# arindamrc/video_analytics

Measured on AMD Instinct MI355X. Metric: clips/sec (224x224, RGB+10-flow two-stream), higher is better.
Workload: dtype f32; 1 GPU; two-stream 224x224, 10-frame TV-L1 flow stack (5 scales x 5 warps x 300 its, fixed), VGG-16 spatial+temporal, batch=32 per GPU; global_batch=32, block_iters=0, tvl1_math=exact, flow_streams=2, batches_in_flight=1, tvl1_params=, tvl1_hip_blob=20e9f45376b19dd960a619139aafc0e8722a8659, parallelism=clips sharded x1, finite=True

## Files before the change

include/va.h:

```cpp
#ifndef VA_H
#define VA_H

#include <stddef.h>
#include <stdint.h>

#ifdef __cplusplus
extern "C" {
#endif

#define VA_OK 0
#define VA_ERR_INVALID 1
#define VA_ERR_HIP 2
#define VA_ERR_WORKSPACE 3
#define VA_ERR_STOPPED 4

#define VA_DTYPE_F32 0
#define VA_DTYPE_BF16 1

typedef struct va_ctx va_ctx;
typedef struct va_vgg16 va_vgg16;

#define VA_VERSION_EXPERIMENTS 0x10000
int va_version(void);
const char* va_last_error(void);
// ... 1 lines not shown
void va_ctx_destroy(va_ctx* ctx);


int va_vgg16_create(va_ctx* ctx, int c_in, int n_classes, int desc_dim, int dtype,
                    const void* const* conv_w, const void* const* conv_b,
                    const void* const* fc_w, const void* const* fc_b,
                    const float* in_mean, const float* in_std,
                    void* stream, va_vgg16** out);
void va_vgg16_destroy(va_vgg16* model);
size_t va_vgg16_workspace_bytes(const va_vgg16* model, int batch);

#define VA_OPT_BF16_VARIANT 1
#define VA_OPT_F32_CONV_KERNEL 2
#define VA_OPT_TRAIN_STOP_AT 3
#define VA_OPT_BF16_FIRST_LAYER 4
int va_vgg16_set_option(va_vgg16* model, int option, int value);

int va_vgg16_forward(va_vgg16* model, const void* x, int x_is_u8, int batch,
                     void* feat, void* desc, void* logits,
                     void* workspace, size_t workspace_bytes, void* stream);

int va_vgg16_classify(va_vgg16* model, const void* feat, int batch, void* desc, void* logits,
                      void* workspace, size_t workspace_bytes, void* stream);

int va_copy_first_layer(va_ctx* ctx, const void* w_rgb, int cout, int n_in, void* w_out, void* stream);

int va_validate_batch(va_ctx* ctx, const void* logits, const void* labels, int batch, int n_classes,
                      void* out, void* stream);


typedef struct va_tvl1_params {
    float tau;
    float lambda;
    float theta;
    int nscales;
// ... 53 lines not shown

int va_flow_motion(va_ctx* ctx, const void* flow, int n_chains, int chain_len, int trajectory, int w, int h,
                   const void* means, void* out, void* stream);

int va_flow_homography(va_ctx* ctx, const void* flow, int n_fields, int w, int h, int iters, double c0_sq, double cmin_sq,
                       void* H, void* stats, void* stream);

int va_flow_compensate(va_ctx* ctx, const void* flow, int n_fields, int w, int h, const void* H, void* out, void* stream);

int va_selftest_exact_math(va_ctx* ctx, float lo, float hi, unsigned long long* mismatches, void* stream);


int va_conv3x3_layer(va_ctx* ctx, int dtype, int kernel_opt, int hw, int cin_pad, int cout, int pool, int linear,
                     int out_f32, int batch, const void* in, const void* w_packed, const float* bias, const float* mask,
                     const void* zeros, void* out, char* kernel_name, int name_len, void* stream);

int va_train_conv_backward_layer(va_ctx* ctx, int kernel_opt, int batch, int hw, int cin, int cin_pad, int cout,
                                 const float* dy, const float* x, float* w_packed, float* bias, float* mom_w, float* mom_b,
                                 float lr, float momentum, float* dx, const float* mask, const float* zeros, float* slab,
                                 float* wt, float* bpart, size_t* scratch_floats, char* info, int info_len, void* stream);
int va_train_fc_backward_layer(va_ctx* ctx, int batch, int out_f, int in_f, const float* dz, const float* x, float* w,
                               float* bias, float* mom_w, float* mom_b, float lr, float momentum, float* dx,
                               const float* mask, float scale, char* info, int info_len, void* stream);
int va_train_pool_layer(va_ctx* ctx, int batch, int hw, int c, const float* y, float* p, const float* dp, float* dy,
                        void* stream);
int va_train_loss(va_ctx* ctx, const float* logits, const void* labels, int n, int k, int c, float* dlogits, float* out,
                  void* stream);
int va_train_loss_multitask(va_ctx* ctx, const float* logits, const void* labels, const void* tasks, int n, int k,
                            int n_heads, const int* head_sizes, float* dlogits, float* out, void* stream);
int va_train_dropout(va_ctx* ctx, float* x, size_t n, unsigned long long dropout_seed, int layer, void* stream);
// ... 54 lines not shown
```

video_analytics_amd/_ffi.py:

```python
import ctypes
import os

_HERE = os.path.dirname(os.path.abspath(__file__))
LIB_PATH = os.path.join(_HERE, "libva_hip.so")

VA_OK, VA_ERR_INVALID, VA_ERR_HIP, VA_ERR_WORKSPACE, VA_ERR_STOPPED = 0, 1, 2, 3, 4
VA_OPT_BF16_VARIANT, VA_OPT_F32_CONV_KERNEL, VA_OPT_TRAIN_STOP_AT, VA_OPT_BF16_FIRST_LAYER = 1, 2, 3, 4

EXPORTS = [
    "va_version", "va_last_error", "va_ctx_create", "va_ctx_destroy",
    "va_vgg16_create", "va_vgg16_destroy", "va_vgg16_workspace_bytes", "va_vgg16_set_option", "va_vgg16_forward", "va_vgg16_classify",
    "va_copy_first_layer", "va_validate_batch",
    "va_tvl1_default_params", "va_tvl1_pyramid_sizes", "va_tvl1_tile_plan", "va_tvl1_workspace_bytes", "va_tvl1_flow",
    "va_flow_to_stack", "va_flow_to_stack_crop", "va_crop_images_u8",
    "va_flow_to_stack_views", "va_crop_images_u8_views", "va_view_mean", "va_flow_field_means", "va_flow_motion",
    "va_selftest_exact_math", "va_tvl1_profile_enable", "va_tvl1_profile_read", "va_tvl1_profile_levels",
    "va_flow_to_stack_snippets", "va_score_consensus", "va_fuse_scores",
    "va_meter_update", "va_meter_average", "va_linear_svm_predict",
    "va_vgg16_train_init", "va_vgg16_train_workspace_bytes", "va_vgg16_train_step",
    "va_vgg16_export_state", "va_vgg16_import_state", "va_vgg16_train_plan",
    "va_conv3x3_layer",
    "va_flow_to_stack_resize", "va_resize_images_u8", "va_vgg16_train_step_consensus",
    "va_flow_homography", "va_flow_compensate",
    "va_rgbdiff_to_stack", "va_fuse_scores_n",
    "va_train_conv_backward_layer", "va_train_fc_backward_layer", "va_train_pool_layer", "va_train_loss", "va_train_dropout",
    "va_vgg16_train_step_multitask", "va_train_loss_multitask",
    "va_linear_svm_fit_workspace_bytes", "va_linear_svm_fit", "va_linear_svm_fit_cg_steps",
]


TUNING_SLOTS = ("stream_levels", "stream_waves", "stream_chunks", "stream_slots", "rows_levels", "stream_ppl",
                "stream_queue", "rows_cfg")
VA_VERSION_EXPERIMENTS = 0x10000


class Tvl1Params(ctypes.Structure):
    _fields_ = [
        ("tau", ctypes.c_float),
        ("lambda_", ctypes.c_float),
        ("theta", ctypes.c_float),
        ("nscales", ctypes.c_int),
        ("warps", ctypes.c_int),
# ... 42 lines not shown
    L.va_last_error.restype = ctypes.c_char_p
    L.va_ctx_create.argtypes = [ci, pp]
    L.va_ctx_create.restype = ci
    L.va_ctx_destroy.argtypes = [vp]
    L.va_ctx_destroy.restype = None
    L.va_vgg16_create.argtypes = [vp, ci, ci, ci, ci, pp, pp, pp, pp, fpp, fpp, vp, pp]
    L.va_vgg16_create.restype = ci
    L.va_vgg16_destroy.argtypes = [vp]
    L.va_vgg16_destroy.restype = None
    L.va_vgg16_workspace_bytes.argtypes = [vp, ci]
    L.va_vgg16_workspace_bytes.restype = sz
    L.va_vgg16_set_option.argtypes = [vp, ci, ci]
    L.va_vgg16_set_option.restype = ci
    L.va_vgg16_forward.argtypes = [vp, vp, ci, ci, vp, vp, vp, vp, sz, vp]
    L.va_vgg16_forward.restype = ci
    L.va_vgg16_classify.argtypes = [vp, vp, ci, vp, vp, vp, sz, vp]
    L.va_vgg16_classify.restype = ci
    L.va_copy_first_layer.argtypes = [vp, vp, ci, ci, vp, vp]
    L.va_copy_first_layer.restype = ci
    L.va_validate_batch.argtypes = [vp, vp, vp, ci, ci, vp, vp]
    L.va_validate_batch.restype = ci
    L.va_tvl1_default_params.argtypes = [ctypes.POINTER(Tvl1Params)]
    L.va_tvl1_default_params.restype = None
    L.va_tvl1_pyramid_sizes.argtypes = [ci, ci, ctypes.POINTER(Tvl1Params), ctypes.POINTER(ci), ctypes.POINTER(ci)]
    L.va_tvl1_pyramid_sizes.restype = ci
    L.va_tvl1_tile_plan.argtypes = [ci, ci, ctypes.POINTER(Tvl1Params), ctypes.POINTER(ci)]
    L.va_tvl1_tile_plan.restype = ci
    L.va_tvl1_workspace_bytes.argtypes = [ci, ci, ci, ci, ctypes.POINTER(Tvl1Params)]
    L.va_tvl1_workspace_bytes.restype = sz
    L.va_tvl1_flow.argtypes = [vp, vp, ci, ci, ci, ci, ci, ctypes.POINTER(Tvl1Params), vp, vp, sz, vp]
# ... 141 lines not shown
```

video_analytics_amd/csrc/vgg.hip:

```cpp
#include "vgg_internal.h"
#include <cstdint>
#include <cstdlib>
#include <cstring>
#include <type_traits>

namespace {

typedef float f32x16 __attribute__((ext_vector_type(16)));
typedef float f32x4 __attribute__((ext_vector_type(4)));
typedef unsigned u32x4 __attribute__((ext_vector_type(4)));

template <int N, typename F>
__device__ __forceinline__ void static_for(F&& f)
{
    if constexpr (N > 0) {
        static_for<N - 1>(f);
        f(std::integral_constant<int, N - 1>{});
    }
}

constexpr int kBK = 16;
constexpr int kLdsStride = 20;


// ... 1571 lines not shown
                } else {
#pragma unroll
                    for (int j = 0; j < 4; ++j) {
                        const int xx = x + (j & 1), yy = y + (j >> 1);
                        if (xx < W && yy < H) {
                            const size_t o = (((size_t)b * H + yy) * W + xx) * a.Cout + n;
                            a.out[o] = (a.mask && !(a.mask[o] > 0.0f)) ? 0.0f : v[j];
                        }
                    }
                }
            }
        }
    }
}



struct FcArgs {
    const float* A;
    const float* Wt;
    float* slab;
    int M, N, K, S, kchunk, Npad;
};

constexpr int kFcDepth = 4;
__global__ void __launch_bounds__(256) k_fc_splitk(FcArgs a)
{
    __shared__ __attribute__((aligned(16))) float sA[2][32 * kLdsStride];
    __shared__ __attribute__((aligned(16))) float sB[2][128 * kLdsStride];
    const int tid = threadIdx.x, lane = tid & 63, wave = tid >> 6;
// ... 225 lines not shown
        VA_LAUNCHED(pool ? "k_conv3x3_mfma<2,2,2,2,true,16>" : "k_conv3x3_mfma<2,2,2,2,false,16>");
    } else {
        a.tiles_n = cout / 64;
        const unsigned grid = (unsigned)(a.tiles_n * a.tiles_x * a.tiles_y * tiles_b);
        if (pool) k_conv3x3_mfma<2, 2, 2, 1, true, 16><<<grid, 256, 0, st>>>(a);
        else k_conv3x3_mfma<2, 2, 2, 1, false, 16><<<grid, 256, 0, st>>>(a);
        VA_LAUNCHED(pool ? "k_conv3x3_mfma<2,2,2,1,true,16>" : "k_conv3x3_mfma<2,2,2,1,false,16>");
    }
    VA_LAUNCH_CHECK();
    return VA_OK;
}

int launch_conv(const ConvLayer& L, const float* zeros, const float* in, float* out, int B, int f32_conv, hipStream_t st)
{
    return launch_conv_ex(L.hw, L.cin_pad, L.cout, L.wp, L.bias, in, out, nullptr, 0, L.pool, B, zeros, f32_conv, st);
}

int launch_conv_bf16(const ConvLayer& L, const __bf16* zeros, int variant, const __bf16* in, void* out, bool out_f32, int B, int n_cu,
                     hipStream_t st, const char** launched = nullptr)
{
    ConvArgsBf a{};
    a.in = in;
    a.zeros = zeros;
    a.taps_x = L.xcol ? 1 : 3;
    a.wp = L.wp_bf;
    a.bias = L.bias;
    a.out = out;
    a.B = B;
    a.H = a.W = L.hw;
    a.Cin = L.cin_pad;
// ... 290 lines not shown
    m->c_in = c_in;
    m->dtype = dtype;
    m->c_in_pad = dtype == VA_DTYPE_BF16 ? 64 : va_cdiv(c_in, VA_CIN_ALIGN) * VA_CIN_ALIGN;
    m->n_classes = n_classes;
    m->desc_dim = desc_dim;
    int hw = 224, cin = c_in, cin_pad = m->c_in_pad;
    int rc = VA_OK;
    auto fail = [&](int code) { va_vgg16_destroy(m); return code; };
    if (hipMalloc(&m->zeros_f32, 512 * sizeof(float)) != hipSuccess || hipMemsetAsync(m->zeros_f32, 0, 512 * sizeof(float), st) != hipSuccess) {
        va_set_error("va_vgg16_create: hipMalloc failed for the zero line");
        return fail(VA_ERR_HIP);
    }
    m->bf16_variant = 0;
    m->bf16_first = 1;
    m->f32_conv = VA_F32_CONV_DEFAULT;
    m->train_stop_at = -1;
    if (dtype == VA_DTYPE_BF16) {
        if (hipMalloc(&m->zeros, 256) != hipSuccess || hipMemsetAsync(m->zeros, 0, 256, st) != hipSuccess) {
            va_set_error("va_vgg16_create: hipMalloc failed for the zero line");
            return fail(VA_ERR_HIP);
        }
    }
    for (int i = 0; i < 13; ++i) {
        ConvLayer& L = m->conv[i];
        L.cin = cin;
        L.cin_pad = cin_pad;
        L.cout = kConvCout[i];
        L.hw = hw;
        L.pool = kConvPool[i];
        const size_t nw = (size_t)L.cout * 9 * L.cin_pad;
        const bool bf = dtype == VA_DTYPE_BF16;
// ... 50 lines not shown
    *out = m;
    return VA_OK;
}

extern "C" void va_vgg16_destroy(va_vgg16* m)
{
    if (!m) return;
    for (int i = 0; i < 13; ++i) {
        if (m->conv[i].wp) (void)hipFree(m->conv[i].wp);
        if (m->conv[i].wp_bf) (void)hipFree(m->conv[i].wp_bf);
        if (m->conv[i].bias) (void)hipFree(m->conv[i].bias);
        if (m->conv[i].mom_w) (void)hipFree(m->conv[i].mom_w);
        if (m->conv[i].mom_b) (void)hipFree(m->conv[i].mom_b);
    }
    if (m->wp_f1) (void)hipFree(m->wp_f1);
    for (int i = 0; i < 4; ++i) {
        if (m->fcw[i]) (void)hipFree(m->fcw[i]);
        if (m->fcb[i]) (void)hipFree(m->fcb[i]);
        if (m->fc_mom_w[i]) (void)hipFree(m->fc_mom_w[i]);
        if (m->fc_mom_b[i]) (void)hipFree(m->fc_mom_b[i]);
    }
    if (m->zeros_f32) (void)hipFree(m->zeros_f32);
    if (m->zeros) (void)hipFree(m->zeros);
    if (m->in_mean) (void)hipFree(m->in_mean);
    if (m->in_std) (void)hipFree(m->in_std);
    delete m;
}

extern "C" size_t va_vgg16_workspace_bytes(const va_vgg16* m, int batch)
{
    if (!m || batch < 1 || batch > 4096) return 0;
    return plan_ws(m, batch).total;
}

extern "C" int va_vgg16_forward(va_vgg16* m, const void* x, int x_is_u8, int batch, void* feat, void* desc, void* logits,
                                void* workspace, size_t workspace_bytes, void* stream)
{
    VA_CHECK_ARG(m != nullptr, "va_vgg16_forward: model is NULL");
    VA_USE_DEVICE(m->ctx);
    VA_CHECK_ARG(x != nullptr && workspace != nullptr, "va_vgg16_forward: NULL input/workspace");
    VA_CHECK_ARG(batch >= 1 && batch <= 4096, "va_vgg16_forward: batch %d out of range [1,4096]", batch);
    VA_CHECK_ARG(!x_is_u8 || (m->in_mean && m->in_std), "va_vgg16_forward: u8 input needs in_mean/in_std at create time");
    VA_CHECK_ARG(((uintptr_t)workspace & 255) == 0, "va_vgg16_forward: workspace must be 256-byte aligned");
    const WsPlan wp = plan_ws(m, batch);
    if (workspace_bytes < wp.total) {
        va_set_error("va_vgg16_forward: workspace too small (%zu < %zu bytes)", workspace_bytes, wp.total);
        return VA_ERR_WORKSPACE;
    }
    hipStream_t st = (hipStream_t)stream;
    char* ws = (char*)workspace;
    float* act[2] = {(float*)(ws + wp.off_act[0]), (float*)(ws + wp.off_act[1])};
    float* slab = (float*)(ws + wp.off_slab);
    float* fcbuf[2] = {(float*)(ws + wp.off_fc[0]), (float*)(ws + wp.off_fc[1])};
    const int B = batch, HW0 = 224 * 224;
// ... 11 lines not shown
        } else if (m->conv[0].xcol) {
            if (x_is_u8)
                k_nchw_to_nhwc_xcol<unsigned char><<<pgrid, 256, 0, st>>>((const unsigned char*)x, (__bf16*)act[1], B, m->c_in, 224, HW0, m->in_mean, m->in_std);
            else
                k_nchw_to_nhwc_xcol<float><<<pgrid, 256, 0, st>>>((const float*)x, (__bf16*)act[1], B, m->c_in, 224, HW0, nullptr, nullptr);
        } else if (x_is_u8)
            k_nchw_to_nhwc_pad<unsigned char, __bf16><<<pgrid, 256, 0, st>>>((const unsigned char*)x, (__bf16*)act[1], B, m->c_in, HW0, m->c_in_pad, m->in_mean, m->in_std);
        else
            k_nchw_to_nhwc_pad<float, __bf16><<<pgrid, 256, 0, st>>>((const float*)x, (__bf16*)act[1], B, m->c_in, HW0, m->c_in_pad, nullptr, nullptr);
        VA_LAUNCH_CHECK();
        for (int i = first; i < 13; ++i) {
            if (int rc = launch_conv_bf16(m->conv[i], m->zeros, m->bf16_variant, (const __bf16*)act[cur], act[cur ^ 1], i == 12, B, m->ctx->n_cu, st)) return rc;
            cur ^= 1;
        }
    } else {
        if (x_is_u8)
            k_nchw_to_nhwc_pad<unsigned char, float><<<pgrid, 256, 0, st>>>((const unsigned char*)x, act[1], B, m->c_in, HW0, m->c_in_pad, m->in_mean, m->in_std);
        else
            k_nchw_to_nhwc_pad<float, float><<<pgrid, 256, 0, st>>>((const float*)x, act[1], B, m->c_in, HW0, m->c_in_pad, nullptr, nullptr);
        VA_LAUNCH_CHECK();
        for (int i = 0; i < 13; ++i) {
            if (int rc = launch_conv(m->conv[i], m->zeros_f32, act[cur], act[cur ^ 1], B, m->f32_conv, st)) return rc;
            cur ^= 1;
        }
    }
    const float* f = act[cur];
    if (feat) {
        const size_t n = (size_t)B * 512 * 49;
        k_nhwc_to_nchw<<<(unsigned)((n + 255) / 256), 256, 0, st>>>(f, (float*)feat, B, 512, 49);
        VA_LAUNCH_CHECK();
    }
    if (desc || logits) return run_classifier(m, f, B, desc, logits, slab, fcbuf, st);
    return VA_OK;
}

extern "C" int va_vgg16_set_option(va_vgg16* m, int option, int value)
{
    VA_CHECK_ARG(m != nullptr, "va_vgg16_set_option: model is NULL");
    switch (option) {
        case VA_OPT_BF16_VARIANT:
            VA_CHECK_ARG((value >= 0 && value <= 2) || (value >= 5 && value <= 7), "va_vgg16_set_option: VA_OPT_BF16_VARIANT must be 0, 1, 2, 5, 6 or 7");
            VA_CHECK_ARG(value != 6 || kVaExperiments, "va_vgg16_set_option: VA_OPT_BF16_VARIANT 6 (k_conv3x3_bpp_bf16) needs a library built with -DVA_EXPERIMENTS");
            m->bf16_variant = value;
            return VA_OK;
        case VA_OPT_BF16_FIRST_LAYER:
            VA_CHECK_ARG(value == 0 || value == 1, "va_vgg16_set_option: VA_OPT_BF16_FIRST_LAYER must be 0 or 1");
            m->bf16_first = value;
            return VA_OK;
        case VA_OPT_F32_CONV_KERNEL:
            VA_CHECK_ARG(value == 0 || value == 1, "va_vgg16_set_option: VA_OPT_F32_CONV_KERNEL must be 0 or 1");
            m->f32_conv = value;
            return VA_OK;
        case VA_OPT_TRAIN_STOP_AT:
            VA_CHECK_ARG(value >= -1 && value <= 12, "va_vgg16_set_option: VA_OPT_TRAIN_STOP_AT must be in [-1,12]");
            m->train_stop_at = value;
            return VA_OK;
        default:
            va_set_error("va_vgg16_set_option: unknown option %d", option);
            return VA_ERR_INVALID;
    }
}

extern "C" int va_vgg16_classify(va_vgg16* m, const void* feat, int batch, void* desc, void* logits, void* workspace,
                                 size_t workspace_bytes, void* stream)
{
    VA_CHECK_ARG(m != nullptr, "va_vgg16_classify: model is NULL");
    VA_USE_DEVICE(m->ctx);
// ... 42 lines not shown
```

video_analytics_amd/csrc/vgg_internal.h:

```cpp
#pragma once
#include "va_internal.h"

struct ConvLayer {
    int cin, cin_pad, cout, hw;
    bool pool;
    bool xcol;
    float* wp;
    __bf16* wp_bf;
    float* bias;
    float* mom_w;
    float* mom_b;
};


struct va_vgg16 {
    va_ctx* ctx;
    int c_in, c_in_pad, n_classes, desc_dim, dtype;
    ConvLayer conv[13];
    float* fcw[4];
    float* fcb[4];
    int fc_in[4], fc_out[4];
    float* in_mean;
    float* in_std;
    __bf16* zeros;
    float* fc_mom_w[4];
    float* fc_mom_b[4];
    float* zeros_f32;
    __bf16* wp_f1;
    int f1_cp, f1_krow;
    int bf16_first;
    int bf16_variant;
    int f32_conv;
    int train_stop_at;
};


int va_conv3x3_f32(int hw, int cin_pad, int cout, const float* wp, const float* bias, const float* in, float* out,
                   const float* mask, int linear, int pool, int B, const float* zeros, int f32_conv, hipStream_t st,
                   const char** launched = nullptr);
int va_fc_f32(const float* A, const float* Wt, const float* bias, float* out, float* slab, int M, int N, int K, int relu, hipStream_t st);
size_t va_fc_slab_floats(int M, int N, int K);
int va_input_to_nhwc_f32(const va_vgg16* m, const void* x, int x_is_u8, int B, float* out, hipStream_t st);

#define VA_MAX_HEADS 8
struct va_heads {
    int n;
    int off[VA_MAX_HEADS + 1];
};
// ... 4 lines not shown
```

video_analytics_amd/pipeline.py:

```python
import torch

from . import flow as vflow
from . import augment, fusion, rgbdiff, synth, vgg, video
from .parameters import (NACTION_CLASSES, NORM_MEANS_TF, NORM_STDS_TF, VIDEO_DESCRIPTOR_DIM,
                         VIDEO_INPUT_FLOW_COUNT)


def build_stream_weights(c_in, seed, device, n_classes=NACTION_CLASSES):
    w = synth.synth_vgg16_weights(c_in=c_in, n_classes=n_classes, desc_dim=VIDEO_DESCRIPTOR_DIM, seed=seed,
                                  device=device)
    if c_in != 3:
        w["conv_w"][0] = vgg.copy_first_layer(w["conv_w"][0].to(device), c_in)
    return w


def check_video(rgb, gray, flow_count, motion, n_snippets, views, consensus, fusion_weights, crops=None):
    if crops is not None:
        raise ValueError("submit_video: a video takes views=, not crops= (one table for all its snippets)")
    if motion != "stack":
        raise ValueError("submit_video: motion=%r is not offered for whole videos (its chains depend on the window); "
                         "use motion='stack'" % (motion,))
    if not isinstance(rgb, torch.Tensor) or rgb.dtype != torch.uint8 or rgb.dim() != 4 or rgb.shape[1] != 3:
        raise ValueError("submit_video: rgb must be a uint8 [T,3,H,W] tensor")
    if not isinstance(gray, torch.Tensor) or gray.dim() != 3 or gray.dtype not in (torch.uint8, torch.float32):
# ... 83 lines not shown

    def _tvl1_frames(self, gray):
        return vflow.bidirectional_sequences(gray) if self.motion == "bidirectional" else gray

    def _camera(self, flow, out):
        if self.camera != "none":
            _, out["homography"], out["camera_share"] = vflow.apply_camera(flow, self.camera, in_place=True)
        return flow

    def _motion_field(self, flow, k):
        if self.motion != "trajectory" and not self.mean_flow:
            return flow
        return vflow.apply_motion(flow, self.L, self.motion, self.mean_flow,
                                  out=self._buffer(self._motion, k, tuple(flow.shape)))

    def _buffer(self, bank, k, shape):
        t = bank[k]
        if t is None or tuple(t.shape) != tuple(shape):
            if t is not None:
                evs = []
                for st in [self._cnn, self._cnn2] + list(vflow.flow_streams(self.device, self.flow_streams)):
                    ev = torch.cuda.Event()
                    ev.record(st)
                    evs.append(ev)
                self._retired.append((t, evs))
            self._retired = [(old, evs) for old, evs in self._retired if not all(e.query() for e in evs)]
            bank[k] = t = torch.empty(shape, dtype=torch.float32, device=self.device)
        return t

    def _check_views(self, rgb, gray, flow_stack, views):
# ... 58 lines not shown
        flow = evs = None
        extra = {}
        if flow_stack is None:
            B, F, H, W = gray.shape
            fbuf = self._buffer(self._flow, k, (B * self.L, 2, H, W))
            flow, evs = vflow.tvl1_flow_concurrent(tv, self.tvl1_params, self.flow_streams, out=fbuf,
                                                   after=[ready, self._flow_read[k]], join=False)
        with torch.cuda.stream(self._cnn):
            self._cnn.wait_event(ready)
            rgb.record_stream(self._cnn)
            _, desc_s, logits_s = self.spatial.forward(rgb if rgb_crops is None else augment.crop_images(rgb, rgb_crops))
            if flow_stack is None:
                for ev in evs:
                    self._cnn.wait_event(ev)
                B, F, H, W = gray.shape
                src = self._motion_field(self._camera(flow, extra), k)
                if flow_crops is None:
                    stack = vflow.flow_to_stack(src, out=self._buffer(self._stack, k, (B, 2 * self.L, H, W)))
                else:
                    stack = vflow.crop_flow_to_stack(src, flow_crops,
                                                     out=self._buffer(self._stack, k, (B, 2 * self.L, 224, 224)),
                                                     invert_x_on_flip=bool(invert_flow_x))
                done = torch.cuda.Event()
                done.record(self._cnn)
                self._flow_read[k] = done
                if self._t_done is not None:
                    self._cnn.wait_event(self._t_done)
                _, desc_t, logits_t = self.temporal.forward(stack)
                self._t_done = torch.cuda.Event()
                self._t_done.record(self._cnn)
            else:
                self._cnn2.wait_event(ready)
                if self._t_done is not None:
                    self._cnn2.wait_event(self._t_done)
                with torch.cuda.stream(self._cnn2):
                    flow_stack.record_stream(self._cnn2)
                    _, desc_t, logits_t = self.temporal.forward(flow_stack)
                    self._t_done = torch.cuda.Event()
                    self._t_done.record(self._cnn2)
                self._cnn.wait_stream(self._cnn2)
            finished = torch.cuda.Event()
            finished.record(self._cnn)
        out = dict(logits_s=logits_s, logits_t=logits_t, desc_s=desc_s, desc_t=desc_t, **extra)
        self._handed_out.extend(out.values())
        out["done"] = finished
# ... 287 lines not shown
```

video_analytics_amd/vgg.py:

```python
import ctypes

import torch

from . import _ffi

_ws_cache = {}


def _workspace(nbytes, device, slot=0):
    key = (device.index, "vgg", slot)
    t = _ws_cache.get(key)
    if t is None or t.numel() < nbytes:
        _ws_cache[key] = t = torch.empty(nbytes, dtype=torch.uint8, device=device)
    return t


def release_workspaces():
    _ws_cache.clear()


def copy_first_layer(w_rgb, n_in):
    if not w_rgb.is_cuda or w_rgb.dtype != torch.float32 or w_rgb.dim() != 4 or tuple(w_rgb.shape[1:]) != (3, 3, 3):
        raise ValueError("copy_first_layer: w_rgb must be a CUDA float32 tensor [Cout,3,3,3]")
    w_rgb = w_rgb.contiguous()
# ... 50 lines not shown
            std = (ctypes.c_float * self.c_in)(*[float(v) for v in in_std])
        h = ctypes.c_void_p()
        with torch.cuda.device(dev):
            _ffi.check(_ffi.lib().va_vgg16_create(_ffi.ctx(dev.index), self.c_in, self.n_classes, self.desc_dim,
                                                  1 if dtype == "bf16" else 0,
                                                  cw, cb, fw, fb, mean, std, _ffi.stream_ptr(self.device), ctypes.byref(h)))
        self._h = h
        del keep

    def _on_my_device(self, t, who):
        if t.device != self.device:
            raise ValueError("Vgg16Stream.%s: tensor is on %s, the model on %s" % (who, t.device, self.device))

    def set_option(self, option, value):
        _ffi.check(_ffi.lib().va_vgg16_set_option(self._h, int(option), int(value)))

    def close(self):
        if getattr(self, "_h", None):
            _ffi.lib().va_vgg16_destroy(self._h)
            self._h = None

    def __del__(self):
        try:
            self.close()
        except Exception:
            pass

    def forward(self, x, want_feat=False):
        if not isinstance(x, torch.Tensor) or not x.is_cuda:
            raise ValueError("Vgg16Stream.forward: x must be a CUDA tensor")
# ... 308 lines not shown
            or tuple(out.shape) != (B, hwo, hwo, cout) or (mask is not None and (mask.dtype != torch.float32
                                                                                 or mask.shape != out.shape))):
        raise ValueError("conv3x3_layer: w_packed / bias / out / mask do not match x")
    if any(not t.is_cuda or t.device != x.device or not t.is_contiguous() for t in tensors):
        raise ValueError("conv3x3_layer: every tensor must be a contiguous tensor on x's device")
    if zeros is None:
        zeros = torch.zeros(256, dtype=torch.uint8, device=x.device)
    name = ctypes.create_string_buffer(128)
    _ffi.check(_ffi.lib().va_conv3x3_layer(
        _ffi.ctx(x.device.index), 1 if bf else 0, int(kernel_opt), hw, cin_pad, cout, int(bool(pool)), int(bool(linear)),
        int(out_f32), B, _ffi.ptr(x), _ffi.ptr(w_packed), _ffi.ptr(bias), _ffi.ptr(mask), _ffi.ptr(zeros), _ffi.ptr(out),
        name, len(name), _ffi.stream_ptr(x.device)))
    return name.value.decode()


def _f32_cuda(who, ref, **tensors):
    for name, t in tensors.items():
        if t is None:
            continue
        if t.dtype != torch.float32 or not t.is_cuda or t.device != ref.device or not t.is_contiguous():
            raise ValueError("%s: %s must be a contiguous float32 tensor on %s" % (who, name, ref.device))


def train_conv_backward_scratch(B, hw, cin, cin_pad, cout, device=None):
    dev = torch.device("cuda", torch.cuda.current_device() if device is None else device)
    need = (ctypes.c_size_t * 3)(0, 0, 0)
    info = ctypes.create_string_buffer(192)
    _ffi.check(_ffi.lib().va_train_conv_backward_layer(
        _ffi.ctx(dev.index), 1, B, hw, cin, cin_pad, cout, None, None, None, None, None, None, 0.0, 0.0, None, None, None, None, None,
        None, need, info, len(info), _ffi.stream_ptr(dev)))
# ... 200 lines not shown
```

Before: 261.9 clips/s.

## Fuse flow quantization, normalization and first VGG conv into one MFMA kernel

Adds a fused first-layer f32 kernel that reads raw NCHW input (flow, u8 or f32), applies the quantize/normalize transform in shared memory, and computes conv1_1 with ReLU using f32 MFMA. The temporal stream now feeds raw flow fields straight into it, skipping the separate flow_to_stack and NCHW-to-NHWC padding passes. This removes the intermediate stack tensor's write and read and the padded-layout conversion. It adds a new kernel path, enabled by default, with its own tiling and numerics that must match the unfused path.

Result: no change. 262.5 clips/s (median of 2 runs) (+0.2%).

```diff
diff --git a/include/va.h b/include/va.h
--- a/include/va.h
+++ b/include/va.h
@@ -39,11 +39,18 @@
 #define VA_OPT_F32_CONV_KERNEL 2
 #define VA_OPT_TRAIN_STOP_AT 3
 #define VA_OPT_BF16_FIRST_LAYER 4
+#define VA_OPT_F32_FIRST_FUSED 5
 int va_vgg16_set_option(va_vgg16* model, int option, int value);
+int va_vgg16_get_option(const va_vgg16* model, int option, int* value);
 
 int va_vgg16_forward(va_vgg16* model, const void* x, int x_is_u8, int batch,
                      void* feat, void* desc, void* logits,
                      void* workspace, size_t workspace_bytes, void* stream);
+
+int va_vgg16_forward_flow(va_vgg16* model, const void* flow, int n_pairs, float bound, float mean, float stdv, int batch,
+                          void* feat, void* desc, void* logits, void* workspace, size_t workspace_bytes, void* stream);
+
+int va_vgg16_first_layer_kernel(const va_vgg16* model, char* kernel_name, int name_len);
 
 int va_vgg16_classify(va_vgg16* model, const void* feat, int batch, void* desc, void* logits,
                       void* workspace, size_t workspace_bytes, void* stream);
@@ -127,6 +134,10 @@
 int va_conv3x3_layer(va_ctx* ctx, int dtype, int kernel_opt, int hw, int cin_pad, int cout, int pool, int linear,
                      int out_f32, int batch, const void* in, const void* w_packed, const float* bias, const float* mask,
                      const void* zeros, void* out, char* kernel_name, int name_len, void* stream);
+
+int va_conv1_fused_layer(va_ctx* ctx, int transform, int hw, int c_in, int cout, int batch, const void* in, const float* w,
+                         const float* bias, const float* mean, const float* stdv, float bound, float qmean, float qstd,
+                         void* out, char* kernel_name, int name_len, void* stream);
 
 int va_train_conv_backward_layer(va_ctx* ctx, int kernel_opt, int batch, int hw, int cin, int cin_pad, int cout,
                                  const float* dy, const float* x, float* w_packed, float* bias, float* mom_w, float* mom_b,
diff --git a/video_analytics_amd/_ffi.py b/video_analytics_amd/_ffi.py
--- a/video_analytics_amd/_ffi.py
+++ b/video_analytics_amd/_ffi.py
@@ -5,7 +5,8 @@
 LIB_PATH = os.path.join(_HERE, "libva_hip.so")
 
 VA_OK, VA_ERR_INVALID, VA_ERR_HIP, VA_ERR_WORKSPACE, VA_ERR_STOPPED = 0, 1, 2, 3, 4
-VA_OPT_BF16_VARIANT, VA_OPT_F32_CONV_KERNEL, VA_OPT_TRAIN_STOP_AT, VA_OPT_BF16_FIRST_LAYER = 1, 2, 3, 4
+VA_OPT_BF16_VARIANT, VA_OPT_F32_CONV_KERNEL, VA_OPT_TRAIN_STOP_AT, VA_OPT_BF16_FIRST_LAYER, VA_OPT_F32_FIRST_FUSED = 1, 2, 3, 4, 5
+VA_XF_FLOW, VA_XF_U8, VA_XF_F32 = 0, 1, 2
 
 EXPORTS = [
     "va_version", "va_last_error", "va_ctx_create", "va_ctx_destroy",
@@ -26,6 +27,7 @@
     "va_train_conv_backward_layer", "va_train_fc_backward_layer", "va_train_pool_layer", "va_train_loss", "va_train_dropout",
     "va_vgg16_train_step_multitask", "va_train_loss_multitask",
     "va_linear_svm_fit_workspace_bytes", "va_linear_svm_fit", "va_linear_svm_fit_cg_steps",
+    "va_vgg16_get_option", "va_vgg16_forward_flow", "va_vgg16_first_layer_kernel", "va_conv1_fused_layer",
 ]
 
 
@@ -98,6 +100,14 @@
     L.va_vgg16_set_option.restype = ci
     L.va_vgg16_forward.argtypes = [vp, vp, ci, ci, vp, vp, vp, vp, sz, vp]
     L.va_vgg16_forward.restype = ci
+    L.va_vgg16_get_option.argtypes = [vp, ci, ctypes.POINTER(ci)]
+    L.va_vgg16_get_option.restype = ci
+    L.va_vgg16_forward_flow.argtypes = [vp, vp, ci, cf, cf, cf, ci, vp, vp, vp, vp, sz, vp]
+    L.va_vgg16_forward_flow.restype = ci
+    L.va_vgg16_first_layer_kernel.argtypes = [vp, ctypes.c_char_p, ci]
+    L.va_vgg16_first_layer_kernel.restype = ci
+    L.va_conv1_fused_layer.argtypes = [vp, ci, ci, ci, ci, ci, vp, vp, vp, vp, vp, cf, cf, cf, vp, ctypes.c_char_p, ci, vp]
+    L.va_conv1_fused_layer.restype = ci
     L.va_vgg16_classify.argtypes = [vp, vp, ci, vp, vp, vp, sz, vp]
     L.va_vgg16_classify.restype = ci
     L.va_copy_first_layer.argtypes = [vp, vp, ci, ci, vp, vp]
diff --git a/video_analytics_amd/csrc/vgg.hip b/video_analytics_amd/csrc/vgg.hip
--- a/video_analytics_amd/csrc/vgg.hip
+++ b/video_analytics_amd/csrc/vgg.hip
@@ -1609,6 +1609,145 @@
     }
 }
 
+enum { VA_XF_FLOW = 0, VA_XF_U8 = 1, VA_XF_F32 = 2 };
+
+struct Conv1F32Args {
+    const void* x;
+    const float* w;
+    const float* bias;
+    float* out;
+    const float* mean;
+    const float* stdv;
+    float bound, qmean, qstd;
+    int B, C, H, W;
+    int tiles_x, tiles_y, ntiles;
+};
+
+template <int XF, int CMAX>
+__global__ void __launch_bounds__(256, CMAX <= 4 ? 4 : 2) k_conv1_fused_f32(Conv1F32Args a)
+{
+    static_assert(CMAX % 2 == 0, "WS = 9 CMAX + 1 must be odd");
+    constexpr int TW = 16, PW = TW + 2, PLANE = PW * PW, WS = 9 * CMAX + 1;
+    typedef typename std::conditional<XF == VA_XF_U8, unsigned char, float>::type TIN;
+    __shared__ float wl[64 * WS];
+    __shared__ float patch[CMAX * PLANE + 1];
+
+    const int tid = threadIdx.x, lane = tid & 63, wave = tid >> 6;
+    const int r31 = lane & 31, hh = lane >> 5;
+    const int C = a.C, H = a.H, W = a.W;
+    const int K = 9 * C, KP = (K + 1) & ~1;
+
+    if (tid == 0) patch[CMAX * PLANE] = 0.0f;
+    for (int i = tid; i < 64 * KP; i += 256) {
+        const int n = i / KP, k = i - n * KP;
+        wl[n * WS + k] = k < K ? a.w[n * K + k] : 0.0f;
+    }
+    int pbase[2];
+#pragma unroll
+    for (int mt = 0; mt < 2; ++mt) {
+        const int m = 64 * wave + 32 * mt + r31;
+        pbase[mt] = (m >> 4) * PW + (m & 15);
+    }
+    const float* const wlane = wl + r31 * WS + hh;
+    const float bias0 = a.bias[r31], bias1 = a.bias[32 + r31];
+
+    for (int tile = blockIdx.x; tile < a.ntiles; tile += gridDim.x) {
+        const int tx = tile % a.tiles_x, ty = (tile / a.tiles_x) % a.tiles_y, b = tile / (a.tiles_x * a.tiles_y);
+        const int X0 = tx * TW, Y0 = ty * TW;
+        __syncthreads();
+        const TIN* const xin = (const TIN*)a.x + (size_t)b * C * H * W;
+        constexpr int U = 4;
+        const int items = C * PLANE;
+        for (int i0 = 0; i0 < items; i0 += 256 * U) {
+            TIN raw[U];
+            bool ok[U];
+            static_for<U>([&](auto I) {
+                constexpr int u = decltype(I)::value;
+                const int i = i0 + u * 256 + tid;
+                const int c = i / PLANE, r = i - c * PLANE, py = r / PW, px = r - py * PW;
+                const int gy = Y0 - 1 + py, gx = X0 - 1 + px;
+                ok[u] = i < items && gy >= 0 && gy < H && gx >= 0 && gx < W;
+                raw[u] = xin[ok[u] ? ((size_t)c * H + gy) * W + gx : 0];
+            });
+            static_for<U>([&](auto I) {
+                constexpr int u = decltype(I)::value;
+                const int i = i0 + u * 256 + tid;
+                float v;
+                if constexpr (XF == VA_XF_FLOW) {
+                    const float t = (255.0f * (raw[u] + a.bound)) / (2.0f * a.bound);
+                    const float q = rintf(fminf(fmaxf(t, 0.0f), 255.0f));
+                    v = (q / 255.0f - a.qmean) / a.qstd;
+                } else if constexpr (XF == VA_XF_U8) {
+                    const int c = i < items ? i / PLANE : 0;
+                    v = ((float)raw[u] / 255.0f - a.mean[c]) / a.stdv[c];
+                } else {
+                    v = raw[u];
+                }
+                if (i < items) patch[i] = ok[u] ? v : 0.0f;
+            });
+        }
+        __syncthreads();
+
+        f32x16 acc[2][2];
+#pragma unroll
+        for (int mt = 0; mt < 2; ++mt)
+#pragma unroll
+            for (int nt = 0; nt < 2; ++nt)
+#pragma unroll
+                for (int r = 0; r < 16; ++r) acc[mt][nt][r] = 0.0f;
+        int c = 0, tap = hh;
+        float fa0, fa1, fb0, fb1;
+#define VA_C1_LOAD(ks_, a0_, a1_, b0_, b1_)                                   \
+    {                                                                         \
+        const bool live_ = 9 * c + tap < K;  \
+        const int ky_ = (tap * 11) >> 5, kx_ = tap - 3 * ky_;                 \
+        const int off_ = c * PLANE + ky_ * PW + kx_;                          \
+        a0_ = patch[live_ ? pbase[0] + off_ : CMAX * PLANE];                  \
+        a1_ = patch[live_ ? pbase[1] + off_ : CMAX * PLANE];                  \
+        b0_ = wlane[2 * (ks_)];                                               \
+        b1_ = wlane[32 * WS + 2 * (ks_)];                                     \
+        tap += 2;                                                             \
+        if (tap >= 9) {                                                       \
+            tap -= 9;                                                         \
+            ++c;                                                              \
+        }                                                                     \
+    }
+        float na0 = 0.0f, na1 = 0.0f, nb0 = 0.0f, nb1 = 0.0f;
+#define VA_C1_MFMA(a0_, a1_, b0_, b1_)                                                     \
+    {                                                                                      \
+        acc[0][0] = __builtin_amdgcn_mfma_f32_32x32x2f32(a0_, b0_, acc[0][0], 0, 0, 0);    \
+        acc[0][1] = __builtin_amdgcn_mfma_f32_32x32x2f32(a0_, b1_, acc[0][1], 0, 0, 0);    \
+        acc[1][0] = __builtin_amdgcn_mfma_f32_32x32x2f32(a1_, b0_, acc[1][0], 0, 0, 0);    \
+        acc[1][1] = __builtin_amdgcn_mfma_f32_32x32x2f32(a1_, b1_, acc[1][1], 0, 0, 0);    \
+    }
+        VA_C1_LOAD(0, fa0, fa1, fb0, fb1)
+        const int NS = KP / 2;
+        for (int ks = 0; ks < NS; ks += 2) {
+            if (ks + 1 < NS) VA_C1_LOAD(ks + 1, na0, na1, nb0, nb1)
+            VA_C1_MFMA(fa0, fa1, fb0, fb1)
+            if (ks + 1 < NS) {
+                if (ks + 2 < NS) VA_C1_LOAD(ks + 2, fa0, fa1, fb0, fb1)
+                VA_C1_MFMA(na0, na1, nb0, nb1)
+            }
+        }
+#undef VA_C1_MFMA
+#undef VA_C1_LOAD
+
+#pragma unroll
+        for (int mt = 0; mt < 2; ++mt)
+#pragma unroll
+            for (int r = 0; r < 16; ++r) {
+                const int m = 64 * wave + 32 * mt + (r & 3) + 8 * (r >> 2) + 4 * hh;
+                const int y = Y0 + (m >> 4), x = X0 + (m & 15);
+                if (x < W && y < H) {
+                    float* const o = a.out + (((size_t)b * H + y) * W + x) * 64 + r31;
+                    o[0] = fmaxf(acc[mt][0][r] + bias0, 0.0f);
+                    o[32] = fmaxf(acc[mt][1][r] + bias1, 0.0f);
+                }
+            }
+    }
+}
+
 
 
 struct FcArgs {
@@ -1864,6 +2003,59 @@
 int launch_conv(const ConvLayer& L, const float* zeros, const float* in, float* out, int B, int f32_conv, hipStream_t st)
 {
     return launch_conv_ex(L.hw, L.cin_pad, L.cout, L.wp, L.bias, in, out, nullptr, 0, L.pool, B, zeros, f32_conv, st);
+}
+
+#ifndef VA_F32_FIRST_FUSED_DEFAULT
+#define VA_F32_FIRST_FUSED_DEFAULT 1
+#endif
+constexpr int kC1MaxCin = 20;
+
+int launch_conv1_fused_f32(int xf, const void* x, const float* w, const float* bias, float* out, const float* mean,
+                           const float* stdv, float bound, float qmean, float qstd, int B, int c_in, int hw, int n_cu,
+                           hipStream_t st, const char** launched = nullptr)
+{
+    if (c_in < 1 || c_in > kC1MaxCin || xf < VA_XF_FLOW || xf > VA_XF_F32) {
+        va_set_error("k_conv1_fused_f32: c_in %d / transform %d unsupported", c_in, xf);
+        return VA_ERR_INVALID;
+    }
+    Conv1F32Args a{};
+    a.x = x;
+    a.w = w;
+    a.bias = bias;
+    a.out = out;
+    a.mean = mean;
+    a.stdv = stdv;
+    a.bound = bound;
+    a.qmean = qmean;
+    a.qstd = qstd;
+    a.B = B;
+    a.C = c_in;
+    a.H = a.W = hw;
+    a.tiles_x = a.tiles_y = va_cdiv(hw, 16);
+    const long nt = (long)a.tiles_x * a.tiles_y * B;
+    if (nt > 0x7fffffffL) {
+        va_set_error("k_conv1_fused_f32: %ld tiles exceed 2^31", nt);
+        return VA_ERR_INVALID;
+    }
+    a.ntiles = (int)nt;
+    const bool small = c_in <= 4;
+    const long resident = (long)(n_cu > 0 ? n_cu : 256) * (small ? 4 : 2);
+    const unsigned grid = (unsigned)(nt < resident ? nt : resident);
+#define VA_LAUNCH_C1(XF_, NAME_, CM_)                                \
+    {                                                                \
+        k_conv1_fused_f32<XF_, CM_><<<grid, 256, 0, st>>>(a);        \
+        VA_LAUNCHED("k_conv1_fused_f32<" #NAME_ "," #CM_ ">");       \
+    }
+    if (xf == VA_XF_FLOW) {
+        if (small) VA_LAUNCH_C1(VA_XF_FLOW, flow, 4) else VA_LAUNCH_C1(VA_XF_FLOW, flow, 20)
+    } else if (xf == VA_XF_U8) {
+        if (small) VA_LAUNCH_C1(VA_XF_U8, u8, 4) else VA_LAUNCH_C1(VA_XF_U8, u8, 20)
+    } else {
+        if (small) VA_LAUNCH_C1(VA_XF_F32, f32, 4) else VA_LAUNCH_C1(VA_XF_F32, f32, 20)
+    }
+#undef VA_LAUNCH_C1
+    VA_LAUNCH_CHECK();
+    return VA_OK;
 }
 
 int launch_conv_bf16(const ConvLayer& L, const __bf16* zeros, int variant, const __bf16* in, void* out, bool out_f32, int B, int n_cu,
@@ -2184,7 +2376,15 @@
     m->bf16_variant = 0;
     m->bf16_first = 1;
     m->f32_conv = VA_F32_CONV_DEFAULT;
+    m->f32_first = VA_F32_FIRST_FUSED_DEFAULT;
     m->train_stop_at = -1;
+    if (dtype == VA_DTYPE_F32 && c_in <= kC1MaxCin) {
+        const size_t nb = (size_t)64 * c_in * 9 * sizeof(float);
+        if (hipMalloc(&m->w1, nb) != hipSuccess || hipMemcpyAsync(m->w1, conv_w[0], nb, hipMemcpyDeviceToDevice, st) != hipSuccess) {
+            va_set_error("va_vgg16_create: hipMalloc failed for the first layer's weights");
+            return fail(VA_ERR_HIP);
+        }
+    }
     if (dtype == VA_DTYPE_BF16) {
         if (hipMalloc(&m->zeros, 256) != hipSuccess || hipMemsetAsync(m->zeros, 0, 256, st) != hipSuccess) {
             va_set_error("va_vgg16_create: hipMalloc failed for the zero line");
@@ -2265,6 +2465,7 @@
         if (m->conv[i].mom_b) (void)hipFree(m->conv[i].mom_b);
     }
     if (m->wp_f1) (void)hipFree(m->wp_f1);
+    if (m->w1) (void)hipFree(m->w1);
     for (int i = 0; i < 4; ++i) {
         if (m->fcw[i]) (void)hipFree(m->fcw[i]);
         if (m->fcb[i]) (void)hipFree(m->fcb[i]);
@@ -2284,11 +2485,10 @@
     return plan_ws(m, batch).total;
 }
 
-extern "C" int va_vgg16_forward(va_vgg16* m, const void* x, int x_is_u8, int batch, void* feat, void* desc, void* logits,
-                                void* workspace, size_t workspace_bytes, void* stream)
-{
-    VA_CHECK_ARG(m != nullptr, "va_vgg16_forward: model is NULL");
-    VA_USE_DEVICE(m->ctx);
+static int vgg16_forward(va_vgg16* m, const void* x, int xf, float bound, float qmean, float qstd, int batch, void* feat,
+                         void* desc, void* logits, void* workspace, size_t workspace_bytes, void* stream)
+{
+    const int x_is_u8 = xf == VA_XF_U8;
     VA_CHECK_ARG(x != nullptr && workspace != nullptr, "va_vgg16_forward: NULL input/workspace");
     VA_CHECK_ARG(batch >= 1 && batch <= 4096, "va_vgg16_forward: batch %d out of range [1,4096]", batch);
     VA_CHECK_ARG(!x_is_u8 || (m->in_mean && m->in_std), "va_vgg16_forward: u8 input needs in_mean/in_std at create time");
@@ -2330,13 +2530,25 @@
             cur ^= 1;
         }
     } else {
-        if (x_is_u8)
-            k_nchw_to_nhwc_pad<unsigned char, float><<<pgrid, 256, 0, st>>>((const unsigned char*)x, act[1], B, m->c_in, HW0, m->c_in_pad, m->in_mean, m->in_std);
-        else
-            k_nchw_to_nhwc_pad<float, float><<<pgrid, 256, 0, st>>>((const float*)x, act[1], B, m->c_in, HW0, m->c_in_pad, nullptr, nullptr);
-        VA_LAUNCH_CHECK();
-        for (int i = 0; i < 13; ++i) {
-            if (int rc = launch_conv(m->conv[i], m->zeros_f32, act[cur], act[cur ^ 1], B, m->f32_conv, st)) return rc;
+        int first = 0;
+        if (m->f32_first == 1 && m->w1 != nullptr) {
+            if (int rc = launch_conv1_fused_f32(xf, x, m->w1, m->conv[0].bias, act[0], m->in_mean, m->in_std, bound, qmean, qstd, B,
+                                                m->c_in, 224, m->ctx->n_cu, st, &m->first_kernel))
+                return rc;
+            first = 1;
+            cur = 0;
+        } else {
+            if (x_is_u8)
+                k_nchw_to_nhwc_pad<unsigned char, float><<<pgrid, 256, 0, st>>>((const unsigned char*)x, act[1], B, m->c_in, HW0, m->c_in_pad, m->in_mean, m->in_std);
+            else
+                k_nchw_to_nhwc_pad<float, float><<<pgrid, 256, 0, st>>>((const float*)x, act[1], B, m->c_in, HW0, m->c_in_pad, nullptr, nullptr);
+            VA_LAUNCH_CHECK();
+        }
+        for (int i = first; i < 13; ++i) {
+            const ConvLayer& L = m->conv[i];
+            if (int rc = launch_conv_ex(L.hw, L.cin_pad, L.cout, L.wp, L.bias, act[cur], act[cur ^ 1], nullptr, 0, L.pool, B, m->zeros_f32,
+                                        m->f32_conv, st, i == 0 ? &m->first_kernel : nullptr))
+                return rc;
             cur ^= 1;
         }
     }
@@ -2348,6 +2560,74 @@
     }
     if (desc || logits) return run_classifier(m, f, B, desc, logits, slab, fcbuf, st);
     return VA_OK;
+}
+
+extern "C" int va_vgg16_forward(va_vgg16* m, const void* x, int x_is_u8, int batch, void* feat, void* desc, void* logits,
+                                void* workspace, size_t workspace_bytes, void* stream)
+{
+    VA_CHECK_ARG(m != nullptr, "va_vgg16_forward: model is NULL");
+    VA_USE_DEVICE(m->ctx);
+    return vgg16_forward(m, x, x_is_u8 ? VA_XF_U8 : VA_XF_F32, 0.0f, 0.0f, 1.0f, batch, feat, desc, logits, workspace, workspace_bytes, stream);
+}
+
+extern "C" int va_vgg16_forward_flow(va_vgg16* m, const void* flow, int n_pairs, float bound, float mean, float stdv, int batch,
+                                     void* feat, void* desc, void* logits, void* workspace, size_t workspace_bytes, void* stream)
+{
+    VA_CHECK_ARG(m != nullptr, "va_vgg16_forward_flow: model is NULL");
+    VA_USE_DEVICE(m->ctx);
+    VA_CHECK_ARG(m->dtype == VA_DTYPE_F32 && m->f32_first == 1 && m->w1 != nullptr,
+                 "va_vgg16_forward_flow: needs an fp32 model with the fused first layer (VA_OPT_F32_FIRST_FUSED = 1, c_in <= %d); "
+                 "use va_flow_to_stack + va_vgg16_forward", kC1MaxCin);
+    VA_CHECK_ARG(bound > 0.0f && stdv > 0.0f, "va_vgg16_forward_flow: bound and std must be > 0");
+    VA_CHECK_ARG(batch >= 1 && m->c_in % 2 == 0 && (long)n_pairs * 2 == (long)batch * m->c_in,
+                 "va_vgg16_forward_flow: %d flow pairs do not make %d stacks of %d planes", n_pairs, batch, m->c_in);
+    return vgg16_forward(m, flow, VA_XF_FLOW, bound, mean, stdv, batch, feat, desc, logits, workspace, workspace_bytes, stream);
+}
+
+extern "C" int va_vgg16_get_option(const va_vgg16* m, int option, int* value)
+{
+    VA_CHECK_ARG(m != nullptr && value != nullptr, "va_vgg16_get_option: NULL argument");
+    switch (option) {
+        case VA_OPT_BF16_VARIANT: *value = m->bf16_variant; return VA_OK;
+        case VA_OPT_BF16_FIRST_LAYER: *value = m->bf16_first; return VA_OK;
+        case VA_OPT_F32_CONV_KERNEL: *value = m->f32_conv; return VA_OK;
+        case VA_OPT_TRAIN_STOP_AT: *value = m->train_stop_at; return VA_OK;
+        case VA_OPT_F32_FIRST_FUSED:
+            *value = m->dtype == VA_DTYPE_F32 && m->f32_first == 1 && m->w1 != nullptr;
+            return VA_OK;
+        default:
+            va_set_error("va_vgg16_get_option: unknown option %d", option);
+            return VA_ERR_INVALID;
+    }
+}
+
+extern "C" int va_vgg16_first_layer_kernel(const va_vgg16* m, char* kernel_name, int name_len)
+{
+    VA_CHECK_ARG(m != nullptr && kernel_name != nullptr && name_len > 0, "va_vgg16_first_layer_kernel: NULL argument");
+    snprintf(kernel_name, (size_t)name_len, "%s", m->first_kernel ? m->first_kernel : "");
+    return VA_OK;
+}
+
+extern "C" int va_conv1_fused_layer(va_ctx* ctx, int transform, int hw, int c_in, int cout, int batch, const void* in,
+                                    const float* w, const float* bias, const float* mean, const float* stdv, float bound,
+                                    float qmean, float qstd, void* out, char* kernel_name, int name_len, void* stream)
+{
+    VA_CHECK_ARG(ctx != nullptr, "va_conv1_fused_layer: ctx is NULL");
+    VA_USE_DEVICE(ctx);
+    if (kernel_name && name_len > 0) kernel_name[0] = 0;
+    VA_CHECK_ARG(in && w && bias && out, "va_conv1_fused_layer: NULL in/w/bias/out");
+    VA_CHECK_ARG(transform >= VA_XF_FLOW && transform <= VA_XF_F32, "va_conv1_fused_layer: transform must be 0 (flow), 1 (u8) or 2 (f32)");
+    VA_CHECK_ARG(transform != VA_XF_U8 || (mean && stdv), "va_conv1_fused_layer: the u8 transform needs mean and std");
+    VA_CHECK_ARG(transform != VA_XF_FLOW || (bound > 0.0f && qstd > 0.0f), "va_conv1_fused_layer: bound and std must be > 0");
+    VA_CHECK_ARG(cout == 64, "va_conv1_fused_layer: cout must be 64 (got %d)", cout);
+    VA_CHECK_ARG(c_in >= 1 && c_in <= kC1MaxCin, "va_conv1_fused_layer: c_in %d out of range [1,%d]", c_in, kC1MaxCin);
+    VA_CHECK_ARG(batch >= 1 && hw >= 1, "va_conv1_fused_layer: batch %d / hw %d < 1", batch, hw);
+    VA_CHECK_ARG((long)batch * hw * hw * 64 < 2147483647L, "va_conv1_fused_layer: %d x %d x %d x 64 activations exceed 2^31 elements", batch, hw, hw);
+    const char* name = nullptr;
+    const int rc = launch_conv1_fused_f32(transform, in, w, bias, (float*)out, mean, stdv, bound, qmean, qstd, batch, c_in, hw, ctx->n_cu,
+                                          (hipStream_t)stream, &name);
+    if (rc == VA_OK && kernel_name && name_len > 0) snprintf(kernel_name, (size_t)name_len, "%s", name ? name : "");
+    return rc;
 }
 
 extern "C" int va_vgg16_set_option(va_vgg16* m, int option, int value)
@@ -2367,6 +2647,10 @@
             VA_CHECK_ARG(value == 0 || value == 1, "va_vgg16_set_option: VA_OPT_F32_CONV_KERNEL must be 0 or 1");
             m->f32_conv = value;
             return VA_OK;
+        case VA_OPT_F32_FIRST_FUSED:
+            VA_CHECK_ARG(value == 0 || value == 1, "va_vgg16_set_option: VA_OPT_F32_FIRST_FUSED must be 0 or 1");
+            m->f32_first = value;
+            return VA_OK;
         case VA_OPT_TRAIN_STOP_AT:
             VA_CHECK_ARG(value >= -1 && value <= 12, "va_vgg16_set_option: VA_OPT_TRAIN_STOP_AT must be in [-1,12]");
             m->train_stop_at = value;
diff --git a/video_analytics_amd/csrc/vgg_internal.h b/video_analytics_amd/csrc/vgg_internal.h
--- a/video_analytics_amd/csrc/vgg_internal.h
+++ b/video_analytics_amd/csrc/vgg_internal.h
@@ -32,6 +32,9 @@
     int bf16_variant;
     int f32_conv;
     int train_stop_at;
+    float* w1;
+    int f32_first;
+    const char* first_kernel;
 };
 
 
diff --git a/video_analytics_amd/pipeline.py b/video_analytics_amd/pipeline.py
--- a/video_analytics_amd/pipeline.py
+++ b/video_analytics_amd/pipeline.py
@@ -121,6 +121,10 @@
         return vflow.apply_motion(flow, self.L, self.motion, self.mean_flow,
                                   out=self._buffer(self._motion, k, tuple(flow.shape)))
 
+    def _flow_direct(self, flow_crops, H, W):
+        return (self.motion == "stack" and not self.mean_flow and self.camera == "none" and flow_crops is None
+                and (H, W) == (224, 224) and self.temporal.takes_flow())
+
     def _buffer(self, bank, k, shape):
         t = bank[k]
         if t is None or tuple(t.shape) != tuple(shape):
@@ -209,21 +213,29 @@
                 for ev in evs:
                     self._cnn.wait_event(ev)
                 B, F, H, W = gray.shape
-                src = self._motion_field(self._camera(flow, extra), k)
-                if flow_crops is None:
-                    stack = vflow.flow_to_stack(src, out=self._buffer(self._stack, k, (B, 2 * self.L, H, W)))
+                if self._flow_direct(flow_crops, H, W):
+                    if self._t_done is not None:
+                        self._cnn.wait_event(self._t_done)
+                    _, desc_t, logits_t = self.temporal.forward_flow(flow, vflow.FLOW_BOUND, NORM_MEANS_TF[0], NORM_STDS_TF[0])
+                    self._t_done = torch.cuda.Event()
+                    self._t_done.record(self._cnn)
+                    self._flow_read[k] = self._t_done
                 else:
-                    stack = vflow.crop_flow_to_stack(src, flow_crops,
-                                                     out=self._buffer(self._stack, k, (B, 2 * self.L, 224, 224)),
-                                                     invert_x_on_flip=bool(invert_flow_x))
-                done = torch.cuda.Event()
-                done.record(self._cnn)
-                self._flow_read[k] = done
-                if self._t_done is not None:
-                    self._cnn.wait_event(self._t_done)
-                _, desc_t, logits_t = self.temporal.forward(stack)
-                self._t_done = torch.cuda.Event()
-                self._t_done.record(self._cnn)
+                    src = self._motion_field(self._camera(flow, extra), k)
+                    if flow_crops is None:
+                        stack = vflow.flow_to_stack(src, out=self._buffer(self._stack, k, (B, 2 * self.L, H, W)))
+                    else:
+                        stack = vflow.crop_flow_to_stack(src, flow_crops,
+                                                         out=self._buffer(self._stack, k, (B, 2 * self.L, 224, 224)),
+                                                         invert_x_on_flip=bool(invert_flow_x))
+                    done = torch.cuda.Event()
+                    done.record(self._cnn)
+                    self._flow_read[k] = done
+                    if self._t_done is not None:
+                        self._cnn.wait_event(self._t_done)
+                    _, desc_t, logits_t = self.temporal.forward(stack)
+                    self._t_done = torch.cuda.Event()
+                    self._t_done.record(self._cnn)
             else:
                 self._cnn2.wait_event(ready)
                 if self._t_done is not None:
diff --git a/video_analytics_amd/vgg.py b/video_analytics_amd/vgg.py
--- a/video_analytics_amd/vgg.py
+++ b/video_analytics_amd/vgg.py
@@ -88,6 +88,42 @@
 
     def set_option(self, option, value):
         _ffi.check(_ffi.lib().va_vgg16_set_option(self._h, int(option), int(value)))
+
+    def get_option(self, option):
+        v = ctypes.c_int(0)
+        _ffi.check(_ffi.lib().va_vgg16_get_option(self._h, int(option), ctypes.byref(v)))
+        return int(v.value)
+
+    def first_layer_kernel(self):
+        name = ctypes.create_string_buffer(128)
+        _ffi.check(_ffi.lib().va_vgg16_first_layer_kernel(self._h, name, len(name)))
+        return name.value.decode()
+
+    def takes_flow(self):
+        return self.dtype == "f32" and self.c_in % 2 == 0 and self.get_option(_ffi.VA_OPT_F32_FIRST_FUSED) == 1
+
+    def forward_flow(self, flow, bound, mean, std):
+        if not isinstance(flow, torch.Tensor) or not flow.is_cuda or flow.dtype != torch.float32:
+            raise ValueError("Vgg16Stream.forward_flow: flow must be a CUDA float32 tensor")
+        half = self.c_in // 2
+        if (flow.dim() != 4 or tuple(flow.shape[1:]) != (2, 224, 224) or self.c_in % 2 or flow.shape[0] < half
+                or flow.shape[0] % half or not flow.is_contiguous()):
+            raise ValueError("Vgg16Stream.forward_flow: flow must be contiguous [B*%d,2,224,224], got %s"
+                             % (max(half, 1), tuple(flow.shape)))
+        self._on_my_device(flow, "forward_flow")
+        if not self.takes_flow():
+            raise ValueError("Vgg16Stream.forward_flow: needs an fp32 model with the fused first layer; use "
+                             "flow.flow_to_stack and forward")
+        N = int(flow.shape[0])
+        B = N // half
+        L = _ffi.lib()
+        ws = _workspace(L.va_vgg16_workspace_bytes(self._h, B), flow.device, self.ws_slot)
+        desc = torch.empty((B, self.desc_dim), dtype=torch.float32, device=flow.device)
+        logits = torch.empty((B, self.n_classes), dtype=torch.float32, device=flow.device)
+        _ffi.check(L.va_vgg16_forward_flow(self._h, _ffi.ptr(flow), N, float(bound), float(mean), float(std), B, None,
+                                           _ffi.ptr(desc), _ffi.ptr(logits), _ffi.ptr(ws), ws.numel(),
+                                           _ffi.stream_ptr(self.device)))
+        return None, desc, logits
 
     def close(self):
         if getattr(self, "_h", None):
@@ -426,6 +462,28 @@
     return name.value.decode()
 
 
+def conv1_fused_layer(x, w, bias, out, transform, mean=None, std=None, bound=0.0, qmean=0.0, qstd=1.0):
+    want = torch.uint8 if transform == _ffi.VA_XF_U8 else torch.float32
+    if x.dtype != want or x.dim() != 4 or x.shape[2] != x.shape[3]:
+        raise ValueError("conv1_fused_layer: x must be %s NCHW [B][c_in][hw][hw]" % want)
+    B, c_in, hw, _ = x.shape
+    cout = w.shape[0]
+    tensors = [x, w, bias, out] + [t for t in (mean, std) if t is not None]
+    if (w.dtype != torch.float32 or tuple(w.shape) != (cout, c_in, 3, 3) or bias.dtype != torch.float32
+            or tuple(bias.shape) != (cout,) or out.dtype != torch.float32 or tuple(out.shape) != (B, hw, hw, cout)):
+        raise ValueError("conv1_fused_layer: w / bias / out do not match x")
+    for t in (mean, std):
+        if t is not None and (t.dtype != torch.float32 or tuple(t.shape) != (c_in,)):
+            raise ValueError("conv1_fused_layer: mean / std must be float32 [c_in]")
+    if any(not t.is_cuda or t.device != x.device or not t.is_contiguous() for t in tensors):
+        raise ValueError("conv1_fused_layer: every tensor must be a contiguous tensor on x's device")
+    name = ctypes.create_string_buffer(128)
+    _ffi.check(_ffi.lib().va_conv1_fused_layer(
+        _ffi.ctx(x.device.index), int(transform), hw, c_in, cout, B, _ffi.ptr(x), _ffi.ptr(w), _ffi.ptr(bias), _ffi.ptr(mean),
+        _ffi.ptr(std), float(bound), float(qmean), float(qstd), _ffi.ptr(out), name, len(name), _ffi.stream_ptr(x.device)))
+    return name.value.decode()
+
+
 def _f32_cuda(who, ref, **tensors):
     for name, t in tensors.items():
         if t is None:
```
